# DistributedSpectrum/TorchPruner

Hardware: AMD Instinct MI355X
Metric: attribution images/sec (whole node) VGG16 Taylor; top-1 retained @ 50% pruned (higher is better)
Workload: dtype fp32

## Files before the change

### csrc/kernels/wino4.hip

```cpp
#include "tp_common.h"

#include <algorithm>
#include <cstdio>
#include <cstdlib>
#include <type_traits>

namespace tp {
namespace w4 {

enum Epi : int { FWD = 0, FWD_POOL = 1, BWD = 2, PARTIAL = 3 };

constexpr int TILES = 32;
constexpr int TK = 32;
constexpr int NPT = 36;
constexpr int U_IMG = NPT * 2 * 16 * 8;
constexpr int U_ROUNDS = U_IMG / 1024;
constexpr int TPL = 16 * 16 + 4;
constexpr unsigned OOB = 0x80000000u;

template <int S> struct Geo;
template <> struct Geo<32> { static constexpr int NI = 1, RH = 18, RWP = 42, IP = 18 * 42; };
template <> struct Geo<16> { static constexpr int NI = 2, RH = 18, RWP = 23, IP = 18 * 23; };
template <> struct Geo<8> { static constexpr int NI = 8, RH = 10, RWP = 14, IP = 146; };
template <> struct Geo<4> { static constexpr int NI = 32, RH = 4, RWP = 4, IP = 17; };
template <int S> constexpr int plane_slots() { return Geo<S>::NI * Geo<S>::IP; }
template <int S, int TB> struct GeoT;
template <int TB> struct GeoT<32, TB> {
  static constexpr int NI = 1, RH = TB / 2 + 2, RWP = 42, IP = (TB / 2 + 2) * 42, PAD = 1;
};
template <int TB> struct GeoT<16, TB> { static constexpr int NI = TB / 16, RH = 18, RWP = 23, IP = 18 * 23, PAD = 1; };
template <int TB> struct GeoT<8, TB> { static constexpr int NI = TB / 4, RH = 10, RWP = 10, IP = 101, PAD = 0; };
template <int TB> struct GeoT<4, TB> { static constexpr int NI = TB, RH = 4, RWP = 4, IP = 17, PAD = 0; };
template <int S> constexpr int x_rounds() { return (2 * plane_slots<S>() + 255) / 256; }
template <int S> struct Band {
  static constexpr bool ON = !(S == 4 || S == 8 || S == 16 || S == 32);
  static constexpr int TPR = (S + 3) / 4, BR = 32 / TPR, TBR = BR * TPR;
  static constexpr int W = 4 * TPR + 2, RWP = W + (W - 1) / 4, RH = 6 * BR;
  static constexpr int NI = 1, IP = RH * RWP, PAD = 1;
  static constexpr int R = (TPR + BR - 2) / BR + 1;
  static_assert(!ON || (S >= 5 && BR >= 1), "band geometry: 5 <= S <= 128");
};

struct Args {
  const float* x;
  const float* u;
  int B, C, K, P;
  int ko;
  long long x_elems;
  const float* scale;
  const float* shift;
  int relu;
  float* out;
  uint8_t* out_argmax;
  const float* act;
  float* taylor;
  float* apoz;
  int tay_mode;
  long long slab;
  int pool_order;
  int dbg;
  const uint8_t* unp;
};

typedef __attribute__((address_space(3))) void* lds_ptr_t;

__device__ __forceinline__ void dma16(__amdgpu_buffer_rsrc_t rs, float* lds_base, unsigned voff, unsigned soff) {
  __builtin_amdgcn_raw_ptr_buffer_load_lds(rs, (lds_ptr_t)lds_base, 16, voff, soff, 0, 0);
}

__device__ __forceinline__ int xcd_remap(int bid, int nwg) {
  const int q = nwg / 8, r = nwg % 8;
  const int xcd = bid % 8, idx = bid / 8;
  return (xcd < r ? xcd * (q + 1) : r * (q + 1) + (xcd - r) * q) + idx;
}

__device__ __forceinline__ void bt6(float& a0, float& a1, float& a2, float& a3, float& a4, float& a5) {
  const float s12 = a1 + a2, s34 = a3 + a4, d12 = a1 - a2, d43 = a4 - a3, d42 = a4 - a2, d31 = a3 - a1;
  const float o0 = fmaf(4.f, a0, fmaf(-5.f, a2, a4));
  const float o5 = fmaf(4.f, a1, fmaf(-5.f, a3, a5));
  a0 = o0;
  a1 = fmaf(-4.f, s12, s34);
  a2 = fmaf(4.f, d12, d43);
  a3 = fmaf(2.f, d31, d42);
  a4 = fmaf(-2.f, d31, d42);
  a5 = o5;
}

__device__ __forceinline__ void input_transform(float (&d)[36]) {
#pragma unroll
  for (int c = 0; c < 6; ++c) bt6(d[c], d[6 + c], d[12 + c], d[18 + c], d[24 + c], d[30 + c]);
#pragma unroll
  for (int r = 0; r < 6; ++r) bt6(d[6 * r], d[6 * r + 1], d[6 * r + 2], d[6 * r + 3], d[6 * r + 4], d[6 * r + 5]);
}

__device__ __forceinline__ void transform_step(float (&d0)[36], float (&d1)[36], int k) {
  float(&d)[36] = (k < 12 ? (k < 6) : (k < 18)) ? d0 : d1;
  if (k < 12) {
    const int c = k % 6;
    bt6(d[c], d[6 + c], d[12 + c], d[18 + c], d[24 + c], d[30 + c]);
  } else {
    const int r = (k - 12) % 6;
    bt6(d[6 * r], d[6 * r + 1], d[6 * r + 2], d[6 * r + 3], d[6 * r + 4], d[6 * r + 5]);
  }
}

__device__ __forceinline__ void at6(const float m0, const float m1, const float m2, const float m3, const float m4,
                                    const float m5, float& y0, float& y1, float& y2, float& y3) {
  const float a = m1 + m2, b = m1 - m2, c = m3 + m4, d = m3 - m4;
  y0 = m0 + a + c;
  y1 = fmaf(2.f, d, b);
  y2 = fmaf(4.f, c, a);
  y3 = fmaf(8.f, d, b) + m5;
}

typedef float f2v __attribute__((ext_vector_type(2)));

__device__ __forceinline__ void at6p(const f2v m0, const f2v m1, const f2v m2, const f2v m3, const f2v m4,
                                     const f2v m5, f2v& y0, f2v& y1, f2v& y2, f2v& y3) {
  const f2v a = m1 + m2, b = m1 - m2, c = m3 + m4, d = m3 - m4;
  y0 = m0 + a + c;
  y1 = 2.f * d + b;
  y2 = 4.f * c + a;
  y3 = 8.f * d + b + m5;
}

__device__ __forceinline__ void output_transform2(const f2v (&m)[36], f2v (&y)[16]) {
  f2v t[24];
#pragma unroll
  for (int c = 0; c < 6; ++c)
    at6p(m[c], m[6 + c], m[12 + c], m[18 + c], m[24 + c], m[30 + c], t[c], t[6 + c], t[12 + c], t[18 + c]);
#pragma unroll
  for (int r = 0; r < 4; ++r)
    at6p(t[6 * r], t[6 * r + 1], t[6 * r + 2], t[6 * r + 3], t[6 * r + 4], t[6 * r + 5], y[4 * r], y[4 * r + 1],
         y[4 * r + 2], y[4 * r + 3]);
}

__device__ __forceinline__ void output_transform(const float (&m)[36], float (&y)[16]) {
  float t[24];
#pragma unroll
  for (int c = 0; c < 6; ++c)
    at6(m[c], m[6 + c], m[12 + c], m[18 + c], m[24 + c], m[30 + c], t[c], t[6 + c], t[12 + c], t[18 + c]);
#pragma unroll
  for (int r = 0; r < 4; ++r)
    at6(t[6 * r], t[6 * r + 1], t[6 * r + 2], t[6 * r + 3], t[6 * r + 4], t[6 * r + 5], y[4 * r], y[4 * r + 1],
        y[4 * r + 2], y[4 * r + 3]);
}

__device__ __forceinline__ void at6row(const f2v* t, f2v& y0, f2v& y1, f2v& y2, f2v& y3) {
  at6p(t[0], t[1], t[2], t[3], t[4], t[5], y0, y1, y2, y3);
}

template <int PH>
__device__ __forceinline__ void sp_partial(const f32x4 (&acc)[NPT], int grp, int lane, float* ya, float* yb) {
  grp &= 1;
  const int j = lane & 15, g = lane >> 4;
#pragma unroll
  for (int nh = 0; nh < 2; ++nh) {
    float* ybuf = nh ? yb : ya;
#pragma unroll
    for (int r = 0; r < 4; r += 2) {
      const int tl = grp * 16 + 4 * g + r;
      f2v m[18];
#pragma unroll
      for (int x = 0; x < 18; ++x) m[x] = f2v{acc[nh * 18 + x][r], acc[nh * 18 + x][r + 1]};
      float* dst = ybuf + tl * TPL + j;
      if constexpr (PH == 0) {
        f2v t0[6], t1[6], t2[6];
#pragma unroll
        for (int c = 0; c < 6; ++c) {
          const f2v a = m[6 + c] + m[12 + c];
          t1[c] = m[6 + c] - m[12 + c];
          t2[c] = a;
          t0[c] = m[c] + a;
        }
        f2v y[12];
        at6row(t0, y[0], y[1], y[2], y[3]);
        at6row(t1, y[4], y[5], y[6], y[7]);
        at6row(t2, y[8], y[9], y[10], y[11]);
#pragma unroll
        for (int q = 0; q < 16; ++q) {
          const f2v v = y[q < 12 ? q : q - 8];
          dst[q * 16] = v.x;
          dst[TPL + q * 16] = v.y;
        }
      } else {
        f2v s[6], d[6];
#pragma unroll
        for (int c = 0; c < 6; ++c) {
          s[c] = m[c] + m[6 + c];
          d[c] = m[c] - m[6 + c];
        }
        f2v ys[4], yd[4], y5[4];
        at6row(s, ys[0], ys[1], ys[2], ys[3]);
        at6row(d, yd[0], yd[1], yd[2], yd[3]);
        at6row(m + 12, y5[0], y5[1], y5[2], y5[3]);
#pragma unroll
        for (int q = 0; q < 16; ++q) {
          const int row = q >> 2, col = q & 3;
          f2v add;
          if (row == 0) add = ys[col];
          else if (row == 1) add = 2.f * yd[col];
          else if (row == 2) add = 4.f * ys[col];
          else add = 8.f * yd[col] + y5[col];
          dst[q * 16] += add.x;
          dst[TPL + q * 16] += add.y;
        }
      }
    }
  }
}

__device__ __forceinline__ void sp_phase1(const f32x4 (&acc)[NPT], int ph, int grp, int lane, float* ya, float* yb,
                                          bool active) {
  if (active && ph == 0) sp_partial<0>(acc, grp, lane, ya, yb);
  __syncthreads();
  if (active && ph == 1) sp_partial<1>(acc, grp, lane, ya, yb);
}

template <int EPI, int S, int NW, int PPW = 1, bool SPP = false>
__device__ __forceinline__ void epilogue(const Args& p, f32x4 (&acc)[PPW][NPT], int t0, int k0, float* ya, float* yb,
                                         float* part) {
  constexpr int TPR = (S + 3) / 4, TI = TPR * TPR;
  constexpr int GROUPS = NW * PPW / 2, TB = 16 * GROUPS, HALVES = TB / 32, TPW = 32 / NW;
  constexpr bool BAND = Band<S>::ON;
  constexpr int TBR = BAND ? Band<S>::TBR : TB;
  constexpr bool PART_TILE = S % 4 != 0;
  static_assert(!BAND || (EPI != FWD_POOL && NW == 4 && PPW == 1), "band geometry: no pooling, 4-wave blocks");
  static_assert(!SPP || PPW == 1, "split-points epilogue: one accumulator set per wave");
  const int tid = threadIdx.x, lane = tid & 63, wave = tid >> 6;
  const int j = lane & 15, g = lane >> 4;
  const bool want_part = EPI == BWD ? p.taylor != nullptr : p.apoz != nullptr;
  const int c4 = lane & 7;
  const int k = k0 + 4 * c4;
  const int KO = p.ko;
  const bool kok = k < KO;
  const float* ysrc = (c4 < 4 ? ya : yb) + (c4 & 3) * 4;
  f32x4 sc4 = {1.f, 1.f, 1.f, 1.f}, sh4 = {0.f, 0.f, 0.f, 0.f};
  if (p.scale && kok) sc4 = *reinterpret_cast<const f32x4*>(p.scale + k);
  if (EPI != BWD && p.shift && kok) sh4 = *reinterpret_cast<const f32x4*>(p.shift + k);

#pragma unroll
  for (int hf = 0; hf < HALVES; ++hf) {
    if constexpr (SPP) sp_phase1(acc[0], wave / GROUPS, wave % GROUPS, lane, ya, yb, (wave % GROUPS) / 2 == hf);
#pragma unroll
    for (int pp = 0; pp < (SPP ? 0 : PPW); ++pp) {
      const int vw = wave + NW * pp, grp = vw % GROUPS, nh = vw / GROUPS;
      if (grp / 2 == hf) {
        float* ybuf = nh ? yb : ya;
#pragma unroll
        for (int r = 0; r < 4; r += 2) {
          const int tl = (grp & 1) * 16 + 4 * g + r;
          f2v m[36], y[16];
#pragma unroll
          for (int x = 0; x < NPT; ++x) m[x] = f2v{acc[pp][x][r], acc[pp][x][r + 1]};
          output_transform2(m, y);
          float* dst = ybuf + tl * TPL + j;
#pragma unroll
          for (int q = 0; q < 16; ++q) {
            dst[q * 16] = y[q].x;
            dst[TPL + q * 16] = y[q].y;
          }
        }
      }
    }
    f32x4 apre[EPI == BWD ? TPW : 1][2];
    if constexpr (EPI == BWD) {
      const int qq = lane >> 3;
#pragma unroll
      for (int tt = 0; tt < TPW; ++tt) {
        const int tbv = hf * 32 + wave * TPW + tt;
        const int pt = t0 + tbv;
        const int b = pt / TI, ti = pt - b * TI, tr = ti / TPR, tc = ti - tr * TPR;
#pragma unroll
        for (int h2 = 0; h2 < 2; ++h2) {
          const int q = qq + 8 * h2;
          const int yy = 4 * tr + (q >> 2), xx = 4 * tc + (q & 3);
          const long long pix = ((long long)b * S + yy) * S + xx;
          const bool ok = kok && pt < p.P && tbv < TBR && (!PART_TILE || (yy < S && xx < S));
          apre[tt][h2] = ok ? *reinterpret_cast<const f32x4*>(p.act + pix * KO + k) : f32x4{0.f, 0.f, 0.f, 0.f};
        }
      }
    }
    __syncthreads();
    if constexpr (EPI == FWD_POOL) {
      const int pp = (lane >> 3) & 3;
      const int py = pp >> 1, px = pp & 1;
#pragma unroll
      for (int tt = 0; tt < TPW / 2; ++tt) {
        const int tl = wave * TPW + 2 * tt + (lane >> 5);
        const int tb = hf * 32 + tl;
        const int pt = t0 + tb;
        f32x4 cnt = {0.f, 0.f, 0.f, 0.f};
        if (pt < p.P) {
          f32x4 best = {0.f, 0.f, 0.f, 0.f};
          unsigned arg = 0;
#pragma unroll
          for (int w = 0; w < 4; ++w) {
            const int q = (2 * py + (w >> 1)) * 4 + 2 * px + (w & 1);
            const f32x4 yv = *reinterpret_cast<const f32x4*>(ysrc + tl * TPL + q * 16);
#pragma unroll
            for (int e = 0; e < 4; ++e) {
              float v = yv[e] * sc4[e] + sh4[e];
              if (p.relu) v = nan_relu(v);
              cnt[e] += v > 0.f ? 1.f : 0.f;
              if (w == 0 || v > best[e] || (v != v && best[e] == best[e])) {
                best[e] = v;
                arg = (arg & ~(0xffu << (8 * e))) | ((unsigned)w << (8 * e));
              }
            }
          }
          const int b = pt / TI, ti = pt - b * TI, tr = ti / TPR, tc = ti - tr * TPR;
          const long long o = (((long long)b * (S / 2) + 2 * tr + py) * (S / 2) + 2 * tc + px) * KO + k;
          if (kok) {
            *reinterpret_cast<f32x4*>(p.out + o) = best;
            *reinterpret_cast<unsigned*>(p.out_argmax + o) = arg;
          }
        }
        if (want_part) {
#pragma unroll
          for (int e = 0; e < 4; ++e) {
            cnt[e] = xsum16(xsum8(cnt[e]));
          }
          if (pp == 0) *reinterpret_cast<f32x4*>(part + tb * TK + 4 * c4) = cnt;
        }
      }
    } else {
      const int qq = lane >> 3;
#pragma unroll
      for (int tt = 0; tt < TPW; ++tt) {
        const int tl = wave * TPW + tt;
        const int tb = hf * 32 + tl;
        const int pt = t0 + tb;
        f32x4 sum = {0.f, 0.f, 0.f, 0.f};
        if (pt < p.P && tb < TBR) {
          const int b = pt / TI, ti = pt - b * TI, tr = ti / TPR, tc = ti - tr * TPR;
#pragma unroll
          for (int h2 = 0; h2 < 2; ++h2) {
            const int q = qq + 8 * h2;
            if (PART_TILE && (4 * tr + (q >> 2) >= S || 4 * tc + (q & 3) >= S)) continue;
            const f32x4 yv = *reinterpret_cast<const f32x4*>(ysrc + tl * TPL + q * 16);
            const long long pix = ((long long)b * S + 4 * tr + (q >> 2)) * S + 4 * tc + (q & 3);
            if constexpr (EPI == PARTIAL) {
              const int yy = 4 * tr + (q >> 2), xx = 4 * tc + (q & 3);
              const long long row = p.pool_order
                                        ? ((((long long)b * (S / 2) + (yy >> 1)) * (S / 2) + (xx >> 1)) * 4 +
                                           (yy & 1) * 2 + (xx & 1))
                                        : pix;
              *reinterpret_cast<f32x4*>(p.out + (long long)blockIdx.y * p.slab + row * p.K + k) = yv;
            } else if constexpr (EPI == FWD) {
              f32x4 v;
#pragma unroll
              for (int e = 0; e < 4; ++e) {
                v[e] = yv[e] * sc4[e] + sh4[e];
                if (p.relu) v[e] = nan_relu(v[e]);
                sum[e] += v[e] > 0.f ? 1.f : 0.f;
              }
              if (kok) *reinterpret_cast<f32x4*>(p.out + pix * KO + k) = v;
            } else {
              const f32x4 a = apre[EPI == BWD ? tt : 0][h2];
#pragma unroll
              for (int e = 0; e < 4; ++e) sum[e] += tay_term(p.tay_mode, yv[e], a[e]);
              if (p.out && kok) {
                f32x4 v;
#pragma unroll
                for (int e = 0; e < 4; ++e) v[e] = a[e] > 0.f ? yv[e] * sc4[e] : 0.f;
                if (p.unp) {
                  const unsigned am4 = *reinterpret_cast<const unsigned*>(p.unp + pix * KO + k);
                  const int yy = 4 * tr + (q >> 2), xx = 4 * tc + (q & 3);
                  const long long o00 = (((long long)b * 2 * S + 2 * yy) * 2 * S + 2 * xx) * KO + k;
#pragma unroll
                  for (int w = 0; w < 4; ++w) {
                    f32x4 o;
#pragma unroll
                    for (int e = 0; e < 4; ++e) o[e] = ((am4 >> (8 * e)) & 0xffu) == (unsigned)w ? v[e] : 0.f;
                    *reinterpret_cast<f32x4*>(p.out + o00 + ((long long)(w >> 1) * 2 * S + (w & 1)) * KO) = o;
                  }
                } else {
                  *reinterpret_cast<f32x4*>(p.out + pix * KO + k) = v;
                }
              }
            }
          }
        }
        if (want_part) {
#pragma unroll
          for (int e = 0; e < 4; ++e) {
            sum[e] = xsum32(xsum16(xsum8(sum[e])));
          }
          if (qq == 0) *reinterpret_cast<f32x4*>(part + tb * TK + 4 * c4) = sum;
        }
      }
    }
    __syncthreads();
  }
  if (!want_part) return;
  if constexpr (BAND) {
    const int b0 = t0 / TI, nimg = (t0 + TBR - 1) / TI - b0 + 1;
    const int blk = t0 / TBR;
    for (int t = tid; t < nimg * TK; t += 64 * NW) {
      const int il = t / TK, kk = t - il * TK;
      const int b = b0 + il;
      if (b >= p.B || k0 + kk >= KO) continue;
      const int s0 = max(0, b * TI - t0), s1 = min(TBR, (b + 1) * TI - t0);
      float s = 0.f;
      for (int ti = s0; ti < s1; ++ti) s += part[ti * TK + kk];
      if constexpr (EPI == BWD) {
        const int slot = blk - (b * TPR) / Band<S>::BR;
        p.taylor[((long long)slot * p.B + b) * KO + k0 + kk] += s;
      } else {
        if (s > 0.f) atomicAdd(p.apoz + (long long)b * KO + k0 + kk, s);
      }
    }
    return;
  }
  constexpr int TIB = TI < TB ? TI : TB;
  constexpr int NIB = TB / TIB;
  const int b0 = t0 / TI;
  for (int t = tid; t < NIB * TK; t += 64 * NW) {
    const int il = t / TK, kk = t - il * TK;
    const int b = b0 + il;
    if (b >= p.B || k0 + kk >= KO) continue;
    float s = 0.f;
    for (int ti = 0; ti < TIB; ++ti) s += part[(il * TIB + ti) * TK + kk];
    constexpr bool split_img = TI > TB;
    if constexpr (EPI == BWD) {
      const int slot = split_img ? (t0 / TB) % (TI / TB) : 0;
      p.taylor[((long long)slot * p.B + b) * KO + k0 + kk] += s;
    } else if constexpr (split_img) {
      if (s > 0.f) atomicAdd(p.apoz + (long long)b * KO + k0 + kk, s);
    } else {
      p.apoz[(long long)b * KO + k0 + kk] += s;
    }
  }
}


typedef int i32x4v __attribute__((ext_vector_type(4)));
__device__ __forceinline__ i32x4v raw_rsrc(const void* base, unsigned bytes) {
  const unsigned long long a = (unsigned long long)base;
  return i32x4v{(int)(unsigned)a, (int)((unsigned)(a >> 32) & 0xffffu), (int)bytes, 0x00020000};
}
__device__ __forceinline__ unsigned lds_addr(const float* p) { return (unsigned)(size_t)(lds_ptr_t)p; }
__device__ __forceinline__ void dma16_asm(const i32x4v& rs, unsigned lds, unsigned voff, unsigned soff) {
  asm volatile("s_mov_b32 m0, %0\n\ts_nop 0\n\tbuffer_load_dwordx4 %1, %2, %3 offen lds"
               :
               : "s"(__builtin_amdgcn_readfirstlane(lds)), "v"(voff), "s"(rs), "s"(soff)
               : "memory", "m0");
}

__device__ __forceinline__ void lds_barrier() {
  asm volatile("s_waitcnt lgkmcnt(0)\n\ts_barrier" ::: "memory");
}

typedef float f2v __attribute__((ext_vector_type(2)));

__device__ __forceinline__ void bt6p(f2v& a0, f2v& a1, f2v& a2, f2v& a3, f2v& a4, f2v& a5) {
  const f2v s12 = a1 + a2, s34 = a3 + a4, d12 = a1 - a2, d43 = a4 - a3, d42 = a4 - a2, d31 = a3 - a1;
  const f2v o0 = 4.f * a0 + (-5.f * a2 + a4);
  const f2v o5 = 4.f * a1 + (-5.f * a3 + a5);
  a0 = o0;
  a1 = -4.f * s12 + s34;
  a2 = 4.f * d12 + d43;
  a3 = 2.f * d31 + d42;
  a4 = -2.f * d31 + d42;
  a5 = o5;
}

#define W4_MFMA2(NOP, c0, c1, a0, a1, w)                                                            \
  asm volatile(NOP                                                                                  \
               "v_mfma_f32_16x16x4_f32 %0, %2, %4, %0\n\t"                                         \
               "v_mfma_f32_16x16x4_f32 %1, %3, %5, %1"                                             \
               : "+v"(c0), "+v"(c1)                                                                 \
               : "v"(a0), "v"(a1), "v"(w.x), "v"(w.y))

__device__ __forceinline__ void bt6q(f2v& a0, f2v& a1, f2v& a2, f2v& a3, f2v& a4, f2v& a5) {
  const f2v p = -4.f * a2 + a4, q = -4.f * a1 + a3, r = a4 - a2, s = a3 - a1;
  const f2v o0 = 4.f * a0 + (-5.f * a2 + a4);
  const f2v o5 = 4.f * a1 + (-5.f * a3 + a5);
  a0 = o0;
  a1 = p + q;
  a2 = p - q;
  a3 = 2.f * s + r;
  a4 = -2.f * s + r;
  a5 = o5;
}

template <int PH>
__device__ __forceinline__ void sp_col(const f2v (&a)[6], f2v (&w)[18], int c) {
  if constexpr (PH == 0) {
    const f2v p = -4.f * a[2] + a[4], q = -4.f * a[1] + a[3];
    w[c] = 4.f * a[0] + (-5.f * a[2] + a[4]);
    w[6 + c] = p + q;
    w[12 + c] = p - q;
  } else {
    const f2v r = a[4] - a[2], s = a[3] - a[1];
    w[c] = 2.f * s + r;
    w[6 + c] = -2.f * s + r;
    w[12 + c] = 4.f * a[1] + (-5.f * a[3] + a[5]);
  }
}

template <int S, typename G, int PH>
__device__ __forceinline__ void sp_read_transform(const float* p0, f2v (&w)[18]) {
  f2v col[2][6];
  auto rd = [&](int q, f2v (&d)[6]) {
#pragma unroll
    for (int r = 0; r < 6; ++r) {
      f2v v = {0.f, 0.f};
      if constexpr (S == 4) {
        if (r >= 1 && r <= 4 && q >= 1 && q <= 4) v = *reinterpret_cast<const f2v*>(p0 + ((r - 1) * 4 + (q - 1)) * 4);
      } else {
        v = *reinterpret_cast<const f2v*>(p0 + (r * G::RWP + q + (G::PAD && q >= 4 ? 1 : 0)) * 4);
      }
      d[r] = v;
      __builtin_amdgcn_sched_barrier(0);
    }
  };
  rd(0, col[0]);
#pragma unroll
  for (int c = 0; c < 6; ++c) {
    if (c + 1 < 6) rd(c + 1, col[(c + 1) & 1]);
    sp_col<PH>(col[c & 1], w, c);
    __builtin_amdgcn_sched_barrier(0);
  }
#pragma unroll
  for (int rr = 0; rr < 3; ++rr) bt6q(w[6 * rr], w[6 * rr + 1], w[6 * rr + 2], w[6 * rr + 3], w[6 * rr + 4], w[6 * rr + 5]);
}

template <typename Mid>
__device__ __forceinline__ void sp_mfma_chunk(int c, int nc, const f2v (&w)[18], const float* ul, f32x4 (&acc)[NPT],
                                              Mid mid, int ph) {
  (void)c;
  (void)nc;
#pragma unroll
  for (int e = 0; e < 2; ++e) {
    if (e == 1) mid();
    const float* ue = ul + (e * 18 + 9 * ph) * 256;
    float2 wq[2][2];
#pragma unroll
    for (int s2 = 0; s2 < 2; ++s2)
#pragma unroll
      for (int h = 0; h < 2; ++h) {
        wq[s2][h] = *reinterpret_cast<const float2*>(ue + s2 * 256 + h * 128);
        __builtin_amdgcn_sched_barrier(0);
      }
#pragma unroll
    for (int i = 0; i < 9; ++i) {
      const float2 w0 = wq[i & 1][0], w1 = wq[i & 1][1];
      if (i + 2 < 9) {
        wq[i & 1][0] = *reinterpret_cast<const float2*>(ue + (i + 2) * 256);
        __builtin_amdgcn_sched_barrier(0);
        wq[i & 1][1] = *reinterpret_cast<const float2*>(ue + (i + 2) * 256 + 128);
        __builtin_amdgcn_sched_barrier(0);
      }
      const int x = 2 * i;
      const float a0 = e ? w[x].y : w[x].x, a1 = e ? w[x + 1].y : w[x + 1].x;
      acc[x] = __builtin_amdgcn_mfma_f32_16x16x4f32(a0, w0.x, acc[x], 0, 0, 0);
      acc[x + 1] = __builtin_amdgcn_mfma_f32_16x16x4f32(a1, w0.y, acc[x + 1], 0, 0, 0);
      acc[18 + x] = __builtin_amdgcn_mfma_f32_16x16x4f32(a0, w1.x, acc[18 + x], 0, 0, 0);
      acc[18 + x + 1] = __builtin_amdgcn_mfma_f32_16x16x4f32(a1, w1.y, acc[18 + x + 1], 0, 0, 0);
      __builtin_amdgcn_sched_barrier(0);
    }
  }
}

template <int EPI, int S, int NW, bool SPREAD = false, bool SPLITP = false>
__global__ __launch_bounds__(64 * NW, 8 / NW) void wino4_m2(Args p) {
  static_assert(!SPREAD || NW == 4, "SPREAD is the 4-wave (two blocks per CU) schedule");
  static_assert(!SPLITP || (NW == 4 && !SPREAD), "split points: 4-wave blocks, burst DMA");
  constexpr int TB = 8 * NW, NG = NW / 2;
  constexpr bool XDBL = NW == 8;
  constexpr bool BAND = Band<S>::ON;
  static_assert(!BAND || SPLITP, "band geometry: the split-points kernel");
  using G = std::conditional_t<BAND, Band<S>, GeoT<S, TB>>;
  constexpr int TPR = (S + 3) / 4, TI = TPR * TPR;
  constexpr int TBR = BAND ? Band<S>::TBR : TB;
  constexpr int PL = G::NI * G::IP;
  constexpr int NXI = (2 * PL + 63) / 64;
  constexpr int KX = (NXI + NW - 1) / NW;
  constexpr int XN = (XDBL ? (NXI > 34 ? NXI : 34) : (NXI > 33 ? NXI : 33)) * 256;
  __shared__ __attribute__((aligned(16))) float us[U_IMG];
  __shared__ __attribute__((aligned(16))) float xs0[XN];
  __shared__ __attribute__((aligned(16))) float xs1[XDBL ? XN : TB * TK];
  static_assert(32 * TPL <= XN && TB * TK <= U_IMG && 32 * TPL <= U_IMG, "epilogue buffers");

  const int tid = threadIdx.x, lane = tid & 63;
  const int wave = __builtin_amdgcn_readfirstlane(tid >> 6);
  const int j = lane & 15, g = lane >> 4;
  const int n_k = p.K / TK;
  const int tile = xcd_remap(blockIdx.x, gridDim.x);
  const int kb = tile % n_k, k0 = kb * TK;
  const int blk_p = tile / n_k;
  const int t0 = blk_p * TBR;
  const int b0 = t0 / TI;
  const int grp = wave % NG, nh = wave / NG;

  const i32x4v urs = raw_rsrc(p.u, (unsigned)((long long)(p.C / 8) * n_k * U_IMG * 4));
  const i32x4v xrs = raw_rsrc(p.x, (unsigned)(p.x_elems * 4));

  const int tib = grp * 16 + j;
  int sbase;
  if constexpr (BAND) {
    const int sl = tib < TBR ? tib : 0;
    sbase = (sl / TPR) * 6 * G::RWP + 5 * (sl % TPR);
  } else {
    const int il = tib / TI, ti = tib - il * TI, tr = ti / TPR, tc = ti - tr * TPR;
    sbase = S == 4 ? il * G::IP : il * G::IP + 4 * tr * G::RWP + (G::PAD ? 5 : 4) * tc;
  }
  const int poff = ((g >> 1) * PL + sbase) * 4 + (g & 1) * 2;

  unsigned xcode[BAND ? KX : (KX + 1) / 2];
#pragma unroll
  for (int i = 0; i < (BAND ? KX : (KX + 1) / 2); ++i) xcode[i] = 0u;
#pragma unroll
  for (int i = 0; i < KX; ++i) {
    const int slot = (wave + NW * i) * 64 + lane;
    const int h = slot / PL, s = slot - h * PL;
    if constexpr (BAND) {
      const int row = s / G::RWP, colp = s - row * G::RWP;
      const int bi = row / 6, rr = row - bi * 6;
      const int blk5 = colp / 5, w5 = colp - blk5 * 5;
      const int xx = 4 * blk5 + w5 - 1;
      const int gr = blk_p * Band<S>::BR + bi;
      const int b = gr / TPR, tr = gr - b * TPR;
      const int yy = 4 * tr - 1 + rr;
      const bool ok = h < 2 && bi < Band<S>::BR && w5 != 4 && xx >= 0 && xx < S && yy >= 0 && yy < S && b < p.B;
      xcode[i] = ok ? 0x80000000u | ((unsigned)h << 30) | (unsigned)(((b - b0) * S + yy) * S + xx) : 0u;
      continue;
    }
    const int im = s / G::IP, rem = s - im * G::IP;
    int xx, yy;
    bool ok;
    if constexpr (S == 4) {
      yy = rem / 4;
      xx = rem - yy * 4;
      ok = rem < 16;
    } else {
      const int row = rem / G::RWP, colp = rem - row * G::RWP;
      int w5 = 0;
      if constexpr (G::PAD) {
        const int blk5 = colp / 5;
        w5 = colp - blk5 * 5;
        xx = 4 * blk5 + w5 - 1;
      } else {
        xx = colp - 1;
      }
      yy = row - 1 + (S == 32 && TB == 32 ? 16 * (blk_p & 1) : 0);
      ok = w5 != 4 && row < G::RH && xx >= 0 && xx < S && yy >= 0 && yy < S;
    }
    ok = ok && h < 2 && im < G::NI && b0 + im < p.B;
    const unsigned code = ok ? (unsigned)((im * S + yy) * S + xx) | ((unsigned)h << 11) | 0x1000u : 0u;
    xcode[i >> 1] |= code << (16 * (i & 1));
  }
  static_assert(BAND || G::NI * S * S <= 2048, "X pixel code");
  const unsigned xbase = (unsigned)b0 * S * S * (unsigned)p.C * 4u;
  const unsigned lane16 = (unsigned)lane * 16u;
  const unsigned c4 = (unsigned)p.C * 4u;

  auto stage_u = [&](int c0, int hf) {
    if (p.dbg & 1) return;
    const unsigned ub = (unsigned)(((c0 >> 3) * n_k + kb) * U_IMG) * 4u;
#pragma unroll
    for (int i = 0; i < (18 + NW - 1) / NW; ++i) {
      const int pt = wave + NW * i;
      if (pt < 18) {
        const int q = hf * 18 + pt;
        dma16_asm(urs, lds_addr(us + q * 256), lane16, ub + (unsigned)q * 1024u);
      }
    }
  };
  auto stage_x = [&](int c0, float* xd) {
    if (p.dbg & 2) return;
#pragma unroll
    for (int i = 0; i < KX; ++i)
      if (wave + NW * i < NXI) {
        unsigned off;
        if constexpr (BAND) {
          const unsigned code = xcode[i];
          off = (code >> 31) ? xbase + (code & 0x3fffffffu) * c4 + ((code >> 26) & 16u) : OOB;
        } else {
          const unsigned code = xcode[i >> 1] >> (16 * (i & 1));
          off = (code & 0x1000u) ? xbase + (code & 0x7ffu) * c4 + ((code >> 7) & 16u) : OOB;
        }
        dma16_asm(xrs, lds_addr(xd + (wave + NW * i) * 256), off, (unsigned)c0 * 4u);
      }
  };
  auto stage_u_piece = [&](int c0, int hf, int i) {
    if (p.dbg & 1) return;
    const int pt = wave + NW * i;
    if (pt < 18) {
      const unsigned ub = (unsigned)(((c0 >> 3) * n_k + kb) * U_IMG) * 4u;
      const int q = hf * 18 + pt;
      dma16_asm(urs, lds_addr(us + q * 256), lane16, ub + (unsigned)q * 1024u);
    }
  };

  const int nc_all = p.C / 8, cps = (nc_all + (int)gridDim.y - 1) / (int)gridDim.y;
  const int c_lo = (int)blockIdx.y * cps, nc = min(nc_all, c_lo + cps);
  f32x4 acc[NPT];
#pragma unroll
  for (int x = 0; x < NPT; ++x) acc[x] = f32x4{0.f, 0.f, 0.f, 0.f};
  const float* ul = us + (SPLITP ? 0 : nh * 128) + j * 8 + 2 * (g ^ ((j >> 3) << 1));
  const bool full_x = (NXI - wave + NW - 1) / NW == KX;
  auto wait_but_x = [&]() {
    if (full_x) asm volatile("s_waitcnt vmcnt(%0)" ::"n"(KX) : "memory");
    else asm volatile("s_waitcnt vmcnt(%0)" ::"n"(KX - 1) : "memory");
  };

  stage_x(8 * c_lo, xs0);
  if (XDBL && c_lo + 1 < nc) stage_x(8 * (c_lo + 1), xs1);
  stage_u(8 * c_lo, 0);
  for (int c = c_lo; c < nc; ++c) {
    float* xb = (XDBL && ((c - c_lo) & 1)) ? xs1 : xs0;
    if (XDBL && c + 1 < nc && c > c_lo) wait_but_x();
    else asm volatile("s_waitcnt vmcnt(0)" ::: "memory");
    lds_barrier();
    stage_u(8 * c, 1);
    if constexpr (SPLITP) {
      f2v w[18];
      if (nh == 0) sp_read_transform<S, G, 0>(xb + poff, w);
      else sp_read_transform<S, G, 1>(xb + poff, w);
      if constexpr (!XDBL) {
        lds_barrier();
        if (c + 1 < nc) stage_x(8 * (c + 1), xs0);
      }
      sp_mfma_chunk(c, nc, w, ul, acc, [&]() {
// ... 367 lines not shown
```

Measured before the change: 227,300.

## Specialize Winograd epilogue on runtime flags and pre-reduce partials per image

Moves the epilogue's second phase into a templated helper specialised at compile time on relu, Taylor mode, output and unpool presence, so the per-element branches are gone. Address arithmetic switches to 32-bit unsigned offsets, and the BWD activation and unpool-argmax prefetch goes through buffer loads with out-of-bounds masking. Partial sums are accumulated across several tiles of the same image in registers before the cross-lane reduction, which shrinks the later shared-memory reduction. The split-point phase now writes both halves in balanced order instead of idling one group per phase. The risks are more template instantiations and code size, and 32-bit offset overflow on large tensors.

```diff
diff --git a/csrc/kernels/wino4.hip b/csrc/kernels/wino4.hip
--- a/csrc/kernels/wino4.hip
+++ b/csrc/kernels/wino4.hip
@@ -150,61 +150,61 @@
   at6p(t[0], t[1], t[2], t[3], t[4], t[5], y0, y1, y2, y3);
 }
 
-template <int PH>
-__device__ __forceinline__ void sp_partial(const f32x4 (&acc)[NPT], int grp, int lane, float* ya, float* yb) {
+template <int PH, int NH, bool ADD>
+__device__ __forceinline__ void sp_partial(const f32x4 (&acc)[NPT], int grp, int lane, float* ybuf) {
   grp &= 1;
   const int j = lane & 15, g = lane >> 4;
 #pragma unroll
-  for (int nh = 0; nh < 2; ++nh) {
-    float* ybuf = nh ? yb : ya;
-#pragma unroll
-    for (int r = 0; r < 4; r += 2) {
-      const int tl = grp * 16 + 4 * g + r;
-      f2v m[18];
-#pragma unroll
-      for (int x = 0; x < 18; ++x) m[x] = f2v{acc[nh * 18 + x][r], acc[nh * 18 + x][r + 1]};
-      float* dst = ybuf + tl * TPL + j;
-      if constexpr (PH == 0) {
-        f2v t0[6], t1[6], t2[6];
-#pragma unroll
-        for (int c = 0; c < 6; ++c) {
-          const f2v a = m[6 + c] + m[12 + c];
-          t1[c] = m[6 + c] - m[12 + c];
-          t2[c] = a;
-          t0[c] = m[c] + a;
-        }
-        f2v y[12];
-        at6row(t0, y[0], y[1], y[2], y[3]);
-        at6row(t1, y[4], y[5], y[6], y[7]);
-        at6row(t2, y[8], y[9], y[10], y[11]);
-#pragma unroll
-        for (int q = 0; q < 16; ++q) {
-          const f2v v = y[q < 12 ? q : q - 8];
-          dst[q * 16] = v.x;
-          dst[TPL + q * 16] = v.y;
-        }
+  for (int r = 0; r < 4; r += 2) {
+    const int tl = grp * 16 + 4 * g + r;
+    f2v m[18];
+#pragma unroll
+    for (int x = 0; x < 18; ++x) m[x] = f2v{acc[NH * 18 + x][r], acc[NH * 18 + x][r + 1]};
+    float* dst = ybuf + tl * TPL + j;
+    f2v out[16];
+    if constexpr (PH == 0) {
+      f2v t0[6], t1[6], t2[6];
+#pragma unroll
+      for (int c = 0; c < 6; ++c) {
+        const f2v a = m[6 + c] + m[12 + c];
+        t1[c] = m[6 + c] - m[12 + c];
+        t2[c] = a;
+        t0[c] = m[c] + a;
+      }
+      f2v y[12];
+      at6row(t0, y[0], y[1], y[2], y[3]);
+      at6row(t1, y[4], y[5], y[6], y[7]);
+      at6row(t2, y[8], y[9], y[10], y[11]);
+#pragma unroll
+      for (int q = 0; q < 16; ++q) out[q] = y[q < 12 ? q : q - 8];
+    } else {
+      f2v s[6], d[6];
+#pragma unroll
+      for (int c = 0; c < 6; ++c) {
+        s[c] = m[c] + m[6 + c];
+        d[c] = m[c] - m[6 + c];
+      }
+      f2v ys[4], yd[4], y5[4];
+      at6row(s, ys[0], ys[1], ys[2], ys[3]);
+      at6row(d, yd[0], yd[1], yd[2], yd[3]);
+      at6row(m + 12, y5[0], y5[1], y5[2], y5[3]);
+#pragma unroll
+      for (int q = 0; q < 16; ++q) {
+        const int row = q >> 2, col = q & 3;
+        if (row == 0) out[q] = ys[col];
+        else if (row == 1) out[q] = 2.f * yd[col];
+        else if (row == 2) out[q] = 4.f * ys[col];
+        else out[q] = 8.f * yd[col] + y5[col];
+      }
+    }
+#pragma unroll
+    for (int q = 0; q < 16; ++q) {
+      if constexpr (ADD) {
+        dst[q * 16] += out[q].x;
+        dst[TPL + q * 16] += out[q].y;
       } else {
-        f2v s[6], d[6];
-#pragma unroll
-        for (int c = 0; c < 6; ++c) {
-          s[c] = m[c] + m[6 + c];
-          d[c] = m[c] - m[6 + c];
-        }
-        f2v ys[4], yd[4], y5[4];
-        at6row(s, ys[0], ys[1], ys[2], ys[3]);
-        at6row(d, yd[0], yd[1], yd[2], yd[3]);
-        at6row(m + 12, y5[0], y5[1], y5[2], y5[3]);
-#pragma unroll
-        for (int q = 0; q < 16; ++q) {
-          const int row = q >> 2, col = q & 3;
-          f2v add;
-          if (row == 0) add = ys[col];
-          else if (row == 1) add = 2.f * yd[col];
-          else if (row == 2) add = 4.f * ys[col];
-          else add = 8.f * yd[col] + y5[col];
-          dst[q * 16] += add.x;
-          dst[TPL + q * 16] += add.y;
-        }
+        dst[q * 16] = out[q].x;
+        dst[TPL + q * 16] = out[q].y;
       }
     }
   }
@@ -212,29 +212,232 @@
 
 __device__ __forceinline__ void sp_phase1(const f32x4 (&acc)[NPT], int ph, int grp, int lane, float* ya, float* yb,
                                           bool active) {
-  if (active && ph == 0) sp_partial<0>(acc, grp, lane, ya, yb);
+  if (active) {
+    if (ph == 0) sp_partial<0, 0, false>(acc, grp, lane, ya);
+    else sp_partial<1, 1, false>(acc, grp, lane, yb);
+  }
   __syncthreads();
-  if (active && ph == 1) sp_partial<1>(acc, grp, lane, ya, yb);
+  if (active) {
+    if (ph == 0) sp_partial<0, 1, true>(acc, grp, lane, yb);
+    else sp_partial<1, 0, true>(acc, grp, lane, ya);
+  }
+}
+
+template <bool PART_, int TAY_, bool RELU_, bool OUT_, bool UNP_>
+struct EpiCfg {
+  static constexpr bool PART = PART_, RELU = RELU_, OUT = OUT_, UNP = UNP_;
+  static constexpr int TAY = TAY_;
+};
+
+template <int S, int NW, int PPW>
+struct EpiGeo {
+  static constexpr int TPR = (S + 3) / 4, TI = TPR * TPR;
+  static constexpr int GROUPS = NW * PPW / 2, TB = 16 * GROUPS, HALVES = TB / 32, TPW = 32 / NW;
+  static constexpr bool BAND = Band<S>::ON;
+  static constexpr int TBR = BAND ? Band<S>::TBR : TB;
+  static constexpr bool PART_TILE = S % 4 != 0;
+  static constexpr int TIB = TI < TB ? TI : TB;
+  static constexpr int NIB = TB / TIB;
+  static constexpr int TPI = BAND ? 1 : (TPW < TIB ? TPW : TIB);
+  static constexpr int SPI = TIB / TPI;
+  static_assert(TPI == 1 || TPI % 2 == 0, "pooled epilogue: a lane pair of tiles lies in one image");
+};
+
+__device__ __forceinline__ float* eptr(float* base, unsigned elem) {
+  return reinterpret_cast<float*>(reinterpret_cast<char*>(base) + elem * 4u);
+}
+
+template <int EPI, int S, int NW, int PPW, typename CF>
+__device__ __forceinline__ void epi_phase2(const Args& p, int hf, int wave, int lane, int t0, int k0, const float* ya,
+                                           const float* yb, float* part, const f32x4 sc4, const f32x4 sh4,
+                                           const f32x4 (&apre)[EPI == BWD ? 32 / NW : 1][2],
+                                           const unsigned (&upre)[EPI == BWD ? 32 / NW : 1][2]) {
+  using E = EpiGeo<S, NW, PPW>;
+  constexpr int TPR = E::TPR, TI = E::TI, TPW = E::TPW, TPI = E::TPI;
+  const int c4 = lane & 7;
+  const int k = k0 + 4 * c4;
+  const unsigned KO = (unsigned)p.ko;
+  const bool kok = k < p.ko;
+  const unsigned b0 = (unsigned)t0 / TI, t0r = (unsigned)t0 % TI;
+  const float* ysrc = (c4 < 4 ? ya : yb) + (c4 & 3) * 4 + wave * (TPW * TPL);
+  const f2v sc01 = {sc4[0], sc4[1]}, sc23 = {sc4[2], sc4[3]}, sh01 = {sh4[0], sh4[1]}, sh23 = {sh4[2], sh4[3]};
+  (void)upre;
+  (void)apre;
+
+  if constexpr (EPI == FWD_POOL) {
+    constexpr int H = S / 2;
+    const int pp = (lane >> 3) & 3;
+    const int py = pp >> 1, px = pp & 1;
+    const int hl = lane >> 5;
+    float* outb = p.out + (long long)b0 * (H * H) * KO;
+    uint8_t* amb = p.out_argmax + (long long)b0 * (H * H) * KO;
+    const unsigned lane_off = (unsigned)(py * H + px + hl * (S == 4 ? H * H : 2)) * KO + (unsigned)k;
+    ysrc += hl * TPL;
+    int cnt[4] = {0, 0, 0, 0};
+#pragma unroll
+    for (int tt = 0; tt < TPW / 2; ++tt) {
+      const int tbe = hf * 32 + wave * TPW + 2 * tt;
+      const unsigned rel = t0r + (unsigned)tbe, bl = rel / TI, ti = rel % TI, tr = ti / TPR, tc = ti % TPR;
+      if (t0 + tbe + hl < p.P) {
+        f32x4 best = {0.f, 0.f, 0.f, 0.f};
+        unsigned ae[4] = {0u, 0u, 0u, 0u};
+#pragma unroll
+        for (int w = 0; w < 4; ++w) {
+          const int q = (2 * py + (w >> 1)) * 4 + 2 * px + (w & 1);
+          const f32x4 yv = *reinterpret_cast<const f32x4*>(ysrc + 2 * tt * TPL + q * 16);
+          const f2v v01 = f2v{yv[0], yv[1]} * sc01 + sh01, v23 = f2v{yv[2], yv[3]} * sc23 + sh23;
+          float v[4] = {v01.x, v01.y, v23.x, v23.y};
+#pragma unroll
+          for (int e = 0; e < 4; ++e) {
+            if constexpr (CF::RELU) v[e] = nan_relu(v[e]);
+            if constexpr (CF::PART) cnt[e] += v[e] > 0.f ? 1 : 0;
+            if (w == 0) {
+              best[e] = v[e];
+            } else {
+              const bool up = !(v[e] <= best[e]) & (best[e] == best[e]);
+              best[e] = up ? v[e] : best[e];
+              ae[e] = up ? (unsigned)w : ae[e];
+            }
+          }
+        }
+        if (kok) {
+          const unsigned o = ((bl * H + 2 * tr) * H + 2 * tc) * KO;
+          *reinterpret_cast<f32x4*>(eptr(outb + o, lane_off)) = best;
+          *reinterpret_cast<unsigned*>(amb + o + lane_off) = ae[0] | (ae[1] << 8) | (ae[2] << 16) | (ae[3] << 24);
+        }
+      }
+      if constexpr (CF::PART) {
+        if (TPI == 1 || (2 * tt + 2) % TPI == 0) {
+          f32x4 c;
+#pragma unroll
+          for (int e = 0; e < 4; ++e) {
+            c[e] = xsum16(xsum8((float)cnt[e]));
+            if (TPI > 1) c[e] = xsum32(c[e]);
+            cnt[e] = 0;
+          }
+          const int slot = TPI == 1 ? tbe + hl : tbe / TPI;
+          if (pp == 0 && (TPI == 1 || hl == 0)) *reinterpret_cast<f32x4*>(part + slot * TK + 4 * c4) = c;
+        }
+      }
+    }
+  } else {
+    const int qq = lane >> 3;
+    const int py = qq >> 2, px = qq & 3;
+    const unsigned lane_off = (unsigned)(py * S + px) * KO + (unsigned)k;
+    const unsigned h2_off = 2u * S * KO;
+    float* outb = nullptr;
+    if constexpr (EPI == FWD || (EPI == BWD && CF::OUT))
+      outb = p.out + (long long)b0 * ((CF::UNP ? 4 : 1) * S * S) * KO;
+    const unsigned lane_off_u = (unsigned)(4 * py * S + 2 * px) * KO + (unsigned)k, h2_off_u = 8u * S * KO;
+    f2v s01 = {0.f, 0.f}, s23 = {0.f, 0.f};
+    float s4[4] = {0.f, 0.f, 0.f, 0.f};
+    int cnt[4] = {0, 0, 0, 0};
+#pragma unroll
+    for (int tt = 0; tt < TPW; ++tt) {
+      const int tb = hf * 32 + wave * TPW + tt;
+      const unsigned rel = t0r + (unsigned)tb, bl = rel / TI, ti = rel % TI, tr = ti / TPR, tc = ti % TPR;
+      if (t0 + tb < p.P && tb < E::TBR) {
+        const unsigned tile_off = ((bl * S + 4 * tr) * S + 4 * tc) * KO;
+#pragma unroll
+        for (int h2 = 0; h2 < 2; ++h2) {
+          if (E::PART_TILE && (4 * (int)tr + py + 2 * h2 >= S || 4 * (int)tc + px >= S)) continue;
+          const f32x4 yv = *reinterpret_cast<const f32x4*>(ysrc + tt * TPL + (qq + 8 * h2) * 16);
+          const f2v y01 = {yv[0], yv[1]}, y23 = {yv[2], yv[3]};
+          if constexpr (EPI == PARTIAL) {
+            const int q = qq + 8 * h2;
+            const int b = (int)(b0 + bl), yy = 4 * (int)tr + (q >> 2), xx = 4 * (int)tc + (q & 3);
+            const long long pix = ((long long)b * S + yy) * S + xx;
+            const long long row = p.pool_order
+                                      ? ((((long long)b * (S / 2) + (yy >> 1)) * (S / 2) + (xx >> 1)) * 4 +
+                                         (yy & 1) * 2 + (xx & 1))
+                                      : pix;
+            *reinterpret_cast<f32x4*>(p.out + (long long)blockIdx.y * p.slab + row * p.K + k) = yv;
+          } else if constexpr (EPI == FWD) {
+            const f2v v01 = y01 * sc01 + sh01, v23 = y23 * sc23 + sh23;
+            f32x4 v = {v01.x, v01.y, v23.x, v23.y};
+#pragma unroll
+            for (int e = 0; e < 4; ++e) {
+              if constexpr (CF::RELU) v[e] = nan_relu(v[e]);
+              if constexpr (CF::PART) cnt[e] += v[e] > 0.f ? 1 : 0;
+            }
+            if (kok) *reinterpret_cast<f32x4*>(eptr(outb + tile_off, lane_off + h2 * h2_off)) = v;
+          } else {
+            const f32x4 a = apre[EPI == BWD ? tt : 0][h2];
+            if constexpr (CF::PART) {
+              if constexpr (CF::TAY == 0) {
+                s01 -= y01 * f2v{a[0], a[1]};
+                s23 -= y23 * f2v{a[2], a[3]};
+              } else {
+#pragma unroll
+                for (int e = 0; e < 4; ++e) s4[e] += CF::TAY == 1 ? fabsf(yv[e]) : (a[e] > 0.f ? fabsf(yv[e]) : 0.f);
+              }
+            }
+            if constexpr (CF::OUT) {
+              if (kok) {
+                const f2v m01 = y01 * sc01, m23 = y23 * sc23;
+                const float m[4] = {m01.x, m01.y, m23.x, m23.y};
+                f32x4 v;
+#pragma unroll
+                for (int e = 0; e < 4; ++e) v[e] = a[e] > 0.f ? m[e] : 0.f;
+                if constexpr (CF::UNP) {
+                  const unsigned am4 = upre[EPI == BWD ? tt : 0][h2];
+                  const unsigned ab[4] = {am4 & 0xffu, (am4 >> 8) & 0xffu, (am4 >> 16) & 0xffu, am4 >> 24};
+                  float* o00 = outb + ((bl * 2 * S + 8 * tr) * 2 * S + 8 * tc) * KO;
+                  const unsigned lo = lane_off_u + h2 * h2_off_u;
+#pragma unroll
+                  for (int w = 0; w < 4; ++w) {
+                    f32x4 o;
+#pragma unroll
+                    for (int e = 0; e < 4; ++e) o[e] = ab[e] == (unsigned)w ? v[e] : 0.f;
+                    *reinterpret_cast<f32x4*>(eptr(o00, lo + (unsigned)((w >> 1) * 2 * S + (w & 1)) * KO)) = o;
+                  }
+                } else {
+                  *reinterpret_cast<f32x4*>(eptr(outb + tile_off, lane_off + h2 * h2_off)) = v;
+                }
+              }
+            }
+          }
+        }
+      }
+      if constexpr (CF::PART) {
+        if ((tt + 1) % TPI == 0) {
+          f32x4 sum;
+          if constexpr (EPI == FWD) sum = f32x4{(float)cnt[0], (float)cnt[1], (float)cnt[2], (float)cnt[3]};
+          else if constexpr (CF::TAY == 0) sum = f32x4{s01.x, s01.y, s23.x, s23.y};
+          else sum = f32x4{s4[0], s4[1], s4[2], s4[3]};
+#pragma unroll
+          for (int e = 0; e < 4; ++e) {
+            sum[e] = xsum32(xsum16(xsum8(sum[e])));
+            cnt[e] = 0;
+            s4[e] = 0.f;
+          }
+          s01 = s23 = f2v{0.f, 0.f};
+          if (qq == 0) *reinterpret_cast<f32x4*>(part + (tb / TPI) * TK + 4 * c4) = sum;
+        }
+      }
+    }
+  }
 }
 
 template <int EPI, int S, int NW, int PPW = 1, bool SPP = false>
 __device__ __forceinline__ void epilogue(const Args& p, f32x4 (&acc)[PPW][NPT], int t0, int k0, float* ya, float* yb,
                                          float* part) {
-  constexpr int TPR = (S + 3) / 4, TI = TPR * TPR;
-  constexpr int GROUPS = NW * PPW / 2, TB = 16 * GROUPS, HALVES = TB / 32, TPW = 32 / NW;
-  constexpr bool BAND = Band<S>::ON;
-  constexpr int TBR = BAND ? Band<S>::TBR : TB;
-  constexpr bool PART_TILE = S % 4 != 0;
+  using E = EpiGeo<S, NW, PPW>;
+  constexpr int TPR = E::TPR, TI = E::TI, GROUPS = E::GROUPS, TB = E::TB, HALVES = E::HALVES;
+  constexpr int TPW = E::TPW;
+  constexpr bool BAND = E::BAND, PART_TILE = E::PART_TILE;
+  constexpr int TBR = E::TBR;
   static_assert(!BAND || (EPI != FWD_POOL && NW == 4 && PPW == 1), "band geometry: no pooling, 4-wave blocks");
   static_assert(!SPP || PPW == 1, "split-points epilogue: one accumulator set per wave");
-  const int tid = threadIdx.x, lane = tid & 63, wave = tid >> 6;
+  int tid = threadIdx.x;
+  asm volatile("" : "+v"(tid));
+  const int lane = tid & 63, wave = __builtin_amdgcn_readfirstlane(tid >> 6);
   const int j = lane & 15, g = lane >> 4;
   const bool want_part = EPI == BWD ? p.taylor != nullptr : p.apoz != nullptr;
   const int c4 = lane & 7;
   const int k = k0 + 4 * c4;
   const int KO = p.ko;
   const bool kok = k < KO;
-  const float* ysrc = (c4 < 4 ? ya : yb) + (c4 & 3) * 4;
   f32x4 sc4 = {1.f, 1.f, 1.f, 1.f}, sh4 = {0.f, 0.f, 0.f, 0.f};
   if (p.scale && kok) sc4 = *reinterpret_cast<const f32x4*>(p.scale + k);
   if (EPI != BWD && p.shift && kok) sh4 = *reinterpret_cast<const f32x4*>(p.shift + k);
@@ -264,131 +467,63 @@
       }
     }
     f32x4 apre[EPI == BWD ? TPW : 1][2];
+    unsigned upre[EPI == BWD ? TPW : 1][2];
     if constexpr (EPI == BWD) {
-      const int qq = lane >> 3;
+      const unsigned elems = (unsigned)p.B * (S * S) * (unsigned)KO;
+      const i32x4 ars = make_rsrc(p.act, elems * 4u), urs = make_rsrc(p.unp, p.unp ? elems : 0u);
+      const bool has_unp = p.out != nullptr && p.unp != nullptr;
+      const int py = lane >> 5, px = (lane >> 3) & 3;
+      const unsigned b0 = (unsigned)t0 / TI, t0r = (unsigned)t0 % TI;
+      const unsigned lane_off = (unsigned)(py * S + px) * (unsigned)KO + (unsigned)k, h2_off = 2u * S * (unsigned)KO;
 #pragma unroll
       for (int tt = 0; tt < TPW; ++tt) {
         const int tbv = hf * 32 + wave * TPW + tt;
-        const int pt = t0 + tbv;
-        const int b = pt / TI, ti = pt - b * TI, tr = ti / TPR, tc = ti - tr * TPR;
+        const unsigned rel = t0r + (unsigned)tbv, bl = rel / TI, ti = rel % TI, tr = ti / TPR, tc = ti % TPR;
+        const bool tile_ok = t0 + tbv < p.P && tbv < TBR;
+        const unsigned tile_off = (((b0 + bl) * S + 4 * tr) * S + 4 * tc) * (unsigned)KO;
 #pragma unroll
         for (int h2 = 0; h2 < 2; ++h2) {
-          const int q = qq + 8 * h2;
-          const int yy = 4 * tr + (q >> 2), xx = 4 * tc + (q & 3);
-          const long long pix = ((long long)b * S + yy) * S + xx;
-          const bool ok = kok && pt < p.P && tbv < TBR && (!PART_TILE || (yy < S && xx < S));
-          apre[tt][h2] = ok ? *reinterpret_cast<const f32x4*>(p.act + pix * KO + k) : f32x4{0.f, 0.f, 0.f, 0.f};
+          const bool ok = kok && tile_ok && (!PART_TILE || (4 * (int)tr + py + 2 * h2 < S && 4 * (int)tc + px < S));
+          const unsigned off = lane_off + h2 * h2_off;
+          apre[tt][h2] = buf_load_f32x4(ars, (int)(ok ? off * 4u : OOB), (int)(tile_off * 4u), 0);
+          upre[tt][h2] = 0u;
+          if (has_unp) upre[tt][h2] = buf_load_u32(urs, (int)(ok ? off : OOB), (int)tile_off, 0);
         }
       }
+    } else {
+      apre[0][0] = apre[0][1] = f32x4{0.f, 0.f, 0.f, 0.f};
+      upre[0][0] = upre[0][1] = 0u;
     }
     __syncthreads();
-    if constexpr (EPI == FWD_POOL) {
-      const int pp = (lane >> 3) & 3;
-      const int py = pp >> 1, px = pp & 1;
-#pragma unroll
-      for (int tt = 0; tt < TPW / 2; ++tt) {
-        const int tl = wave * TPW + 2 * tt + (lane >> 5);
-        const int tb = hf * 32 + tl;
-        const int pt = t0 + tb;
-        f32x4 cnt = {0.f, 0.f, 0.f, 0.f};
-        if (pt < p.P) {
-          f32x4 best = {0.f, 0.f, 0.f, 0.f};
-          unsigned arg = 0;
-#pragma unroll
-          for (int w = 0; w < 4; ++w) {
-            const int q = (2 * py + (w >> 1)) * 4 + 2 * px + (w & 1);
-            const f32x4 yv = *reinterpret_cast<const f32x4*>(ysrc + tl * TPL + q * 16);
-#pragma unroll
-            for (int e = 0; e < 4; ++e) {
-              float v = yv[e] * sc4[e] + sh4[e];
-              if (p.relu) v = nan_relu(v);
-              cnt[e] += v > 0.f ? 1.f : 0.f;
-              if (w == 0 || v > best[e] || (v != v && best[e] == best[e])) {
-                best[e] = v;
-                arg = (arg & ~(0xffu << (8 * e))) | ((unsigned)w << (8 * e));
-              }
-            }
-          }
-          const int b = pt / TI, ti = pt - b * TI, tr = ti / TPR, tc = ti - tr * TPR;
-          const long long o = (((long long)b * (S / 2) + 2 * tr + py) * (S / 2) + 2 * tc + px) * KO + k;
-          if (kok) {
-            *reinterpret_cast<f32x4*>(p.out + o) = best;
-            *reinterpret_cast<unsigned*>(p.out_argmax + o) = arg;
-          }
+    auto run = [&](auto cf) {
+      epi_phase2<EPI, S, NW, PPW, decltype(cf)>(p, hf, wave, lane, t0, k0, ya, yb, part, sc4, sh4, apre, upre);
+    };
+    if constexpr (EPI == PARTIAL) {
+      run(EpiCfg<false, 0, false, true, false>{});
+    } else if constexpr (EPI == BWD) {
+      auto by_out = [&](auto pc, auto tc) {
+        constexpr bool PT = decltype(pc)::value;
+        constexpr int TM = decltype(tc)::value;
+        if (p.out == nullptr) {
+          if constexpr (PT) run(EpiCfg<PT, TM, false, false, false>{});
+        } else if (!BAND && p.unp != nullptr) {
+          if constexpr (!BAND) run(EpiCfg<PT, TM, false, true, true>{});
+        } else {
+          run(EpiCfg<PT, TM, false, true, false>{});
         }
-        if (want_part) {
-#pragma unroll
-          for (int e = 0; e < 4; ++e) {
-            cnt[e] = xsum16(xsum8(cnt[e]));
-          }
-          if (pp == 0) *reinterpret_cast<f32x4*>(part + tb * TK + 4 * c4) = cnt;
-        }
-      }
+      };
+      using std::integral_constant;
+      if (!want_part) by_out(std::false_type{}, integral_constant<int, 0>{});
+      else if (p.tay_mode == 1) by_out(std::true_type{}, integral_constant<int, 1>{});
+      else if (p.tay_mode == 2) by_out(std::true_type{}, integral_constant<int, 2>{});
+      else by_out(std::true_type{}, integral_constant<int, 0>{});
     } else {
-      const int qq = lane >> 3;
-#pragma unroll
-      for (int tt = 0; tt < TPW; ++tt) {
-        const int tl = wave * TPW + tt;
-        const int tb = hf * 32 + tl;
-        const int pt = t0 + tb;
-        f32x4 sum = {0.f, 0.f, 0.f, 0.f};
-        if (pt < p.P && tb < TBR) {
-          const int b = pt / TI, ti = pt - b * TI, tr = ti / TPR, tc = ti - tr * TPR;
-#pragma unroll
-          for (int h2 = 0; h2 < 2; ++h2) {
-            const int q = qq + 8 * h2;
-            if (PART_TILE && (4 * tr + (q >> 2) >= S || 4 * tc + (q & 3) >= S)) continue;
-            const f32x4 yv = *reinterpret_cast<const f32x4*>(ysrc + tl * TPL + q * 16);
-            const long long pix = ((long long)b * S + 4 * tr + (q >> 2)) * S + 4 * tc + (q & 3);
-            if constexpr (EPI == PARTIAL) {
-              const int yy = 4 * tr + (q >> 2), xx = 4 * tc + (q & 3);
-              const long long row = p.pool_order
-                                        ? ((((long long)b * (S / 2) + (yy >> 1)) * (S / 2) + (xx >> 1)) * 4 +
-                                           (yy & 1) * 2 + (xx & 1))
-                                        : pix;
-              *reinterpret_cast<f32x4*>(p.out + (long long)blockIdx.y * p.slab + row * p.K + k) = yv;
-            } else if constexpr (EPI == FWD) {
-              f32x4 v;
-#pragma unroll
-              for (int e = 0; e < 4; ++e) {
-                v[e] = yv[e] * sc4[e] + sh4[e];
-                if (p.relu) v[e] = nan_relu(v[e]);
-                sum[e] += v[e] > 0.f ? 1.f : 0.f;
-              }
-              if (kok) *reinterpret_cast<f32x4*>(p.out + pix * KO + k) = v;
-            } else {
-              const f32x4 a = apre[EPI == BWD ? tt : 0][h2];
-#pragma unroll
-              for (int e = 0; e < 4; ++e) sum[e] += tay_term(p.tay_mode, yv[e], a[e]);
-              if (p.out && kok) {
-                f32x4 v;
-#pragma unroll
-                for (int e = 0; e < 4; ++e) v[e] = a[e] > 0.f ? yv[e] * sc4[e] : 0.f;
-                if (p.unp) {
-                  const unsigned am4 = *reinterpret_cast<const unsigned*>(p.unp + pix * KO + k);
-                  const int yy = 4 * tr + (q >> 2), xx = 4 * tc + (q & 3);
-                  const long long o00 = (((long long)b * 2 * S + 2 * yy) * 2 * S + 2 * xx) * KO + k;
-#pragma unroll
-                  for (int w = 0; w < 4; ++w) {
-                    f32x4 o;
-#pragma unroll
-                    for (int e = 0; e < 4; ++e) o[e] = ((am4 >> (8 * e)) & 0xffu) == (unsigned)w ? v[e] : 0.f;
-                    *reinterpret_cast<f32x4*>(p.out + o00 + ((long long)(w >> 1) * 2 * S + (w & 1)) * KO) = o;
-                  }
-                } else {
-                  *reinterpret_cast<f32x4*>(p.out + pix * KO + k) = v;
-                }
-              }
-            }
-          }
-        }
-        if (want_part) {
-#pragma unroll
-          for (int e = 0; e < 4; ++e) {
-            sum[e] = xsum32(xsum16(xsum8(sum[e])));
-          }
-          if (qq == 0) *reinterpret_cast<f32x4*>(part + tb * TK + 4 * c4) = sum;
-        }
+      if (want_part) {
+        if (p.relu) run(EpiCfg<true, 0, true, true, false>{});
+        else run(EpiCfg<true, 0, false, true, false>{});
+      } else {
+        if (p.relu) run(EpiCfg<false, 0, true, true, false>{});
+        else run(EpiCfg<false, 0, false, true, false>{});
       }
     }
     __syncthreads();
@@ -413,15 +548,15 @@
     }
     return;
   }
-  constexpr int TIB = TI < TB ? TI : TB;
-  constexpr int NIB = TB / TIB;
+  constexpr int NIB = E::NIB, SPI = E::SPI;
   const int b0 = t0 / TI;
   for (int t = tid; t < NIB * TK; t += 64 * NW) {
     const int il = t / TK, kk = t - il * TK;
     const int b = b0 + il;
     if (b >= p.B || k0 + kk >= KO) continue;
     float s = 0.f;
-    for (int ti = 0; ti < TIB; ++ti) s += part[(il * TIB + ti) * TK + kk];
+#pragma unroll
+    for (int si = 0; si < SPI; ++si) s += part[(il * SPI + si) * TK + kk];
     constexpr bool split_img = TI > TB;
     if constexpr (EPI == BWD) {
       const int slot = split_img ? (t0 / TB) % (TI / TB) : 0;
```

After: 234,400 (median of 6 runs). 1.03x the previous value.
